# microsoft/OmniParser

Hardware: AMD Instinct MI355X
Metric: screenshots/sec end-to-end (detect+caption) @1920x1080 (higher is better)
Workload: dtype f32 (split-f16x3 MFMA)

## Files before the change

### omniparser_amd/csrc/gemm_dma.hip

```cpp
#include "omni_internal.h"
#include "gemm_common.h"
#include <string.h>
#include <type_traits>

OMNI_RANGE_GUARD_TU()

namespace {

typedef __attribute__((address_space(3))) void lds_void;

struct GemmArgs {
  const unsigned char* x; const unsigned char* w; const float* bias; const float* res; unsigned char* y;
  int M, N, K, nk;
  int ldi, in_coff, ldo, out_coff, ldr, res_coff;
  int mtiles, ntiles, xcd_order, xcd_n;
  float oscale;
  int img_tiles; unsigned w_img_stride; const float* img_oscale;
};

#if defined(__AMDGCN__)
struct RowBuf {
  __amdgpu_buffer_rsrc_t r;
  __device__ __forceinline__ RowBuf(const void* base, unsigned bytes) : r(__builtin_amdgcn_make_buffer_rsrc((void*)base, 0, (int)bytes, 0x00020000)) {}
  __device__ __forceinline__ void store16(unsigned off, f32x4 v) const { __builtin_amdgcn_raw_buffer_store_b128(__builtin_bit_cast(u32x4, v), r, (int)off, 0, 0); }
  __device__ __forceinline__ f32x4 load16(unsigned off) const { return __builtin_bit_cast(f32x4, __builtin_amdgcn_raw_buffer_load_b128(r, (int)off, 0, 0)); }
};
#else
struct RowBuf {
  unsigned char* base; unsigned bytes;
  RowBuf(const void* b, unsigned n) : base((unsigned char*)b), bytes(n) {}
  void store16(unsigned off, f32x4 v) const { if (off + 16u <= bytes) *reinterpret_cast<f32x4*>(base + off) = v; }
  f32x4 load16(unsigned off) const { return off + 16u <= bytes ? *reinterpret_cast<const f32x4*>(base + off) : f32x4{0.f, 0.f, 0.f, 0.f}; }
};
#endif

template <int BM, int BN, int WM, int WN, int TM, int TN, int LDS_BYTES, int ACT, bool OSPLIT, bool RES>
__device__ __forceinline__ void gemm_epilogue(f32x16 (&acc)[TM][TN], const GemmArgs& a, unsigned char* lds, int m0, int n0, int wave, int lane, float osc) {
  constexpr int NW = WM * WN;
  const int wm = wave / WN, wn = wave % WN;
  const int hsel = lane >> 5;
  static_assert(TN % 2 == 0, "epilogue stages 64 channels (256 bytes per row) of a wave at a time");
  constexpr int EP = 272;
  static_assert(NW * 32 * EP <= LDS_BYTES, "epilogue staging must fit the LDS ring");
  __syncthreads();
  unsigned char* stg = lds + wave * (32 * EP);
  float amax = 0.0f;
  const int rrow = lane >> 4, chunk = lane & 15;
  const int trows = min(a.M - m0, BM), wc0 = n0 + wn * (BN / WN);
  const RowBuf ybuf(a.y + ((long long)m0 * a.ldo + a.out_coff + wc0) * 4, (unsigned)(trows - 1) * (unsigned)(a.ldo * 4) + (BN / WN) * 4);
  const RowBuf rbuf(RES ? reinterpret_cast<const unsigned char*>(a.res) + ((long long)m0 * a.ldr + a.res_coff + wc0) * 4 : a.y,
// ... 36 lines not shown
            for (int c = 0; c < 4; c += 2) {
              f32x2 t = __builtin_elementwise_fma(f32x2{ac[q * 4 + c], ac[q * 4 + c + 1]}, (f32x2)osc, f32x2{bq[j][q][c], bq[j][q][c + 1]});
              if constexpr (ACT == OMNI_ACT_SILU) t = f32x2{t[0] / (1.0f + expf(-t[0])), t[1] / (1.0f + expf(-t[1]))};
              v[c] = t[0]; v[c + 1] = t[1];
            }
          }
          const int cl = j * 32 + q * 8 + 4 * hsel;
          if constexpr (OSPLIT) {
            uint2 hi, lo;
            omni_split4(v, hi, lo, amax);
            *reinterpret_cast<uint2*>(wr + omni_split_off(cl)) = hi;
            *reinterpret_cast<uint2*>(wr + omni_split_off(cl) + 32) = lo;
          } else {
            *reinterpret_cast<f32x4*>(wr + cl * 4) = f32x4{v[0], v[1], v[2], v[3]};
          }
        }
      OMNI_WAVE_SYNC();
      f32x4 ov[8];
#pragma unroll
      for (int it = 0; it < 8; ++it) {
        ov[it] = *reinterpret_cast<const f32x4*>(stg + (it * 4 + rrow) * EP + chunk * 16);
        if constexpr (RES) ov[it] += rres[it];
      }
      if constexpr (RES) { if (i + 1 < TM) load_res(i + 1); }
#pragma unroll
      for (int it = 0; it < 8; ++it) ybuf.store16(yoff + (unsigned)(i * 32 + it * 4) * (unsigned)(a.ldo * 4) + jh * 256, ov[it]);
      OMNI_WAVE_SYNC();
      __builtin_amdgcn_sched_barrier(0);
    }
  }
  if constexpr (OSPLIT) omni_report_range(amax);
}

template <int BM, int BN, int WM, int WN, int NSTAGE, int ACT, bool OSPLIT, bool RES, int SCHED = 0>
__global__ __launch_bounds__(WM * WN * 64, 2) void gemm_dma_kernel(GemmArgs a) {
#if defined(__HIP_DEVICE_COMPILE__)
  constexpr int NW = WM * WN;
  constexpr int TM = BM / (32 * WM), TN = BN / (32 * WN);
  constexpr int A_DMA = BM / (8 * NW), B_DMA = BN / (8 * NW);
  constexpr int DPS = A_DMA + B_DMA;
  constexpr int STAGE = (BM + BN) * 128;
  constexpr int NP = TM / 2;
  constexpr int NU = 2 * NP;
  constexpr int NM = 6 * TN;
  static_assert(TM % 2 == 0 && TN >= 1 && A_DMA >= 1 && B_DMA >= 1 && NSTAGE >= 2 && NSTAGE <= 4, "tile / wave grid mismatch");
  static_assert(BM * 128 + (TN - 1) * 4096 < 65536 && (TM - 1) * 4096 < 65536, "ds_read immediate offsets");
  __shared__ __attribute__((aligned(16))) unsigned char lds[NSTAGE * STAGE];

  const int tid = threadIdx.x, lane = tid & 63;
  const int wave = __builtin_amdgcn_readfirstlane(tid >> 6);
  const int wm = wave / WN, wn = wave % WN;
  int mt, nt;
  if (!tile_of_block(blockIdx.x, a.mtiles, a.ntiles, a.xcd_order, a.xcd_n, mt, nt)) return;
  const int m0 = __builtin_amdgcn_readfirstlane(mt) * BM, n0 = __builtin_amdgcn_readfirstlane(nt) * BN;
  const int img = a.img_tiles ? __builtin_amdgcn_readfirstlane(mt / a.img_tiles) : 0;
  const float osc = a.img_oscale ? a.img_oscale[img] : a.oscale;

  const int rsub = lane >> 3, slot = lane & 7;
  unsigned voffA[A_DMA], voffB[B_DMA];
  auto pieceA = [&](int i) { return SCHED == 2 ? wave + NW * i : wave * A_DMA + i; };
#pragma unroll
  for (int i = 0; i < A_DMA; ++i) {
    const int rl = pieceA(i) * 8 + rsub;
    const int rr = min(rl, a.M - 1 - m0);
    voffA[i] = (unsigned)rr * (unsigned)(a.ldi * 4) + (unsigned)((slot ^ ((rl >> 1) & 7)) * 16);
  }
#pragma unroll
  for (int i = 0; i < B_DMA; ++i) {
    const int rl = (wave * B_DMA + i) * 8 + rsub;
    const int rr = min(rl, a.N - 1 - n0);
    voffB[i] = (unsigned)rr * (unsigned)(a.K * 4) + (unsigned)((slot ^ ((rl >> 1) & 7)) * 16);
  }
  const __amdgpu_buffer_rsrc_t rsrcA =
      __builtin_amdgcn_make_buffer_rsrc((void*)(a.x + ((long long)m0 * a.ldi + a.in_coff) * 4), 0, 0x7fffffff, 0x00020000);
  const __amdgpu_buffer_rsrc_t rsrcB =
      __builtin_amdgcn_make_buffer_rsrc((void*)(a.w + (long long)img * a.w_img_stride + (long long)n0 * a.K * 4), 0, 0x7fffffff, 0x00020000);
  auto issue_piece = [&](int kt, int stage, int i) {
    const int so = kt * 128;
    if (i < A_DMA)
      __builtin_amdgcn_raw_ptr_buffer_load_lds(rsrcA, (lds_void*)(lds + stage * STAGE + pieceA(i) * 1024), 16, voffA[i], so, 0, 0);
    else
      __builtin_amdgcn_raw_ptr_buffer_load_lds(rsrcB, (lds_void*)(lds + stage * STAGE + BM * 128 + (wave * B_DMA + i - A_DMA) * 1024), 16,
                                               voffB[i - A_DMA], so, 0, 0);
  };
  auto issue = [&](int kt, int stage) {
#pragma unroll
    for (int i = 0; i < DPS; ++i) issue_piece(kt, stage, i);
  };

  const int swz = (lane >> 1) & 7, hsel = lane >> 5;
  int offA[4], offW[4];
#pragma unroll
  for (int gp = 0; gp < 4; ++gp) {
    const int c = ((((gp >> 1) * 4 + (gp & 1) * 2 + hsel) ^ swz)) * 16;
    offA[gp] = (wm * (BM / WM) + (lane & 31)) * 128 + c;
    offW[gp] = BM * 128 + (wn * (BN / WN) + (lane & 31)) * 128 + c;
  }
  struct AF { f16x8 h[2], l[2]; };
  struct WF { f16x8 h[TN], l[TN]; };
  auto loadA = [&](const unsigned char* st, int g, int ip, AF& f) {
#pragma unroll
    for (int t = 0; t < 2; ++t) {
      f.h[t] = *reinterpret_cast<const f16x8*>(st + offA[g * 2 + 0] + (ip * 2 + t) * 4096);
      f.l[t] = *reinterpret_cast<const f16x8*>(st + offA[g * 2 + 1] + (ip * 2 + t) * 4096);
    }
  };
  auto loadW = [&](const unsigned char* st, int g, WF& f) {
#pragma unroll
    for (int j = 0; j < TN; ++j) {
      f.h[j] = *reinterpret_cast<const f16x8*>(st + offW[g * 2 + 0] + j * 4096);
      f.l[j] = *reinterpret_cast<const f16x8*>(st + offW[g * 2 + 1] + j * 4096);
    }
  };

  f32x16 acc[TM][TN];
#pragma unroll
  for (int i = 0; i < TM; ++i)
#pragma unroll
    for (int j = 0; j < TN; ++j)
#pragma unroll
// ... 30 lines not shown
    constexpr bool MORE = decltype(more_tag)::value;
    if constexpr (NSTAGE > 2 && MORE) OMNI_WAIT_VMCNT((NSTAGE - 2) * DPS);
    else OMNI_WAIT_VMCNT(0);
    __builtin_amdgcn_s_barrier();
    const unsigned char* st = lds + stage * STAGE;
    loadW(st, 0, wf[0]);
    loadA(st, 0, 0, af[0]);
#pragma unroll
    for (int u = 0; u < NU; ++u) {
      const int g = u / NP, ip = u % NP;
      int nds = 0;
      if (u + 1 < NU) {
        const int g2 = (u + 1) / NP, ip2 = (u + 1) % NP;
        if (g2 != g) { loadW(st, g2, wf[g2 & 1]); nds += 2 * TN; }
        loadA(st, g2, ip2, af[(u + 1) & 1]);
        nds += 4;
      }
      if constexpr (MORE) {
#pragma unroll
        for (int i = u * PPU; i < (u + 1) * PPU && i < DPS; ++i) issue_piece(kt + NSTAGE - 1, nstage, i);
      }
      mma(af[u & 1], wf[g & 1], ip);
      {
        const int npc = (MORE && u < IU) ? PPU : 0;
#pragma unroll
        for (int k = 0; k < NM; ++k) {
          __builtin_amdgcn_sched_group_barrier(0x8, 1, 0);
          if (k < nds) __builtin_amdgcn_sched_group_barrier(0x100, 1, 0);
          else if (k < nds + npc) __builtin_amdgcn_sched_group_barrier(0x20, 1, 0);
        }
      }
      __builtin_amdgcn_sched_barrier(0);
    }
    stage = stage + 1 == NSTAGE ? 0 : stage + 1;
    nstage = nstage + 1 == NSTAGE ? 0 : nstage + 1;
  };
  if constexpr (SCHED == 2) {
    static_assert(BM == 256 && BN == 256 && WM == 2 && WN == 4 && NSTAGE == 2 && TM == 4 && TN == 2 && A_DMA == 4 && B_DMA == 4, "ping-pong: 256x256 tile, 8 waves");
    OMNI_WAIT_VMCNT(0);
    __builtin_amdgcn_s_barrier();
    if (wm == 1) __builtin_amdgcn_s_barrier();
    auto phase_barrier = [&]() {
      __builtin_amdgcn_sched_barrier(0);
      __builtin_amdgcn_s_barrier();
      __builtin_amdgcn_sched_barrier(0);
    };
    {
      AF afp;
      auto slice_pp = [&](int kt, auto more_tag) {
        constexpr bool MORE = decltype(more_tag)::value;
        const unsigned char* st = lds + stage * STAGE;
#pragma unroll
        for (int u = 0; u < 4; ++u) {
          const int g = u & 1, ip = u >> 1;
          if (u < 2) loadW(st, g, wf[g]);
          loadA(st, g, ip, afp);
          if constexpr (MORE) {
            if (u == 0) { issue_piece(kt + 1, nstage, 0); issue_piece(kt + 1, nstage, 2); }
            if (u == 1) { issue_piece(kt + 1, nstage, A_DMA + 0); issue_piece(kt + 1, nstage, A_DMA + 1); }
            if (u == 2) { issue_piece(kt + 1, nstage, A_DMA + 2); issue_piece(kt + 1, nstage, A_DMA + 3); }
            if (u == 3) { issue_piece(kt + 1, nstage, 1); issue_piece(kt + 1, nstage, 3); }
            if (u == 1) OMNI_WAIT_VMCNT(4);
            if (u == 3) OMNI_WAIT_VMCNT(2);
          } else {
            if (u == 1) OMNI_WAIT_VMCNT(0);
          }
          phase_barrier();
          __builtin_amdgcn_s_setprio(1);
          mma(afp, wf[g], ip);
          __builtin_amdgcn_s_setprio(0);
          phase_barrier();
        }
        stage ^= 1;
        nstage ^= 1;
      };
      int ktp = 0;
      for (; ktp + 1 < nk; ++ktp) slice_pp(ktp, std::true_type{});
      for (; ktp < nk; ++ktp) slice_pp(ktp, std::false_type{});
    }
    if (wm == 0) __builtin_amdgcn_s_barrier();
  } else {
  int kt = 0;
  for (; kt + NSTAGE - 1 < nk; ++kt) slice(kt, std::true_type{});
  for (; kt < nk; ++kt) slice(kt, std::false_type{});
  }

  gemm_epilogue<BM, BN, WM, WN, TM, TN, NSTAGE * STAGE, ACT, OSPLIT, RES>(acc, a, lds, m0, n0, wave, lane, osc);
#endif
}

__global__ __launch_bounds__(256) void split_convert_kernel(const float* __restrict__ x, unsigned char* __restrict__ y, long long rows,
                                                            int C, int ldi, int in_coff, int ldo, int out_coff) {
  const int gpr = C / 16;
  const long long idx = (long long)blockIdx.x * blockDim.x + threadIdx.x;
  if (idx >= rows * gpr) return;
  const long long r = idx / gpr;
  const int g = (int)(idx - r * gpr);
  const float* src = x + r * ldi + in_coff + g * 16;
  f32x4 v[4];
#pragma unroll
  for (int q = 0; q < 4; ++q) v[q] = *reinterpret_cast<const f32x4*>(src + q * 4);
  uint2 hi[4], lo[4];
#pragma unroll
  for (int q = 0; q < 4; ++q) {
    float t[4] = {v[q][0], v[q][1], v[q][2], v[q][3]};
// ... 111 lines not shown
        float v[4];
#pragma unroll
        for (int r = 0; r < 4; r += 2) {
          const f32x2 t = omni_gelu2(__builtin_elementwise_fma(f32x2{a1[0][q * 4 + r], a1[0][q * 4 + r + 1]} + f32x2{a1[1][q * 4 + r], a1[1][q * 4 + r + 1]},
                                                               (f32x2)osc1, f32x2{bq[r], bq[r + 1]}));
          v[r] = t[0]; v[r + 1] = t[1];
        }
        omni_split4(v, hq[qq], lq[qq], amax);
      }
      gh[kg] = __builtin_bit_cast(f16x8, u32x4{hq[0].x, hq[0].y, hq[1].x, hq[1].y});
      gl[kg] = __builtin_bit_cast(f16x8, u32x4{lq[0].x, lq[0].y, lq[1].x, lq[1].y});
    }
#pragma unroll
    for (int kg = 0; kg < 2; ++kg)
#pragma unroll
      for (int j = 0; j < OB; j += 2) {
        const unsigned char* sw = st + W1B + j * 4096;
        const f16x8 wh0 = *reinterpret_cast<const f16x8*>(sw + fo[kg][0]), wl0 = *reinterpret_cast<const f16x8*>(sw + fo[kg][1]);
        const f16x8 wh1 = *reinterpret_cast<const f16x8*>(sw + 4096 + fo[kg][0]), wl1 = *reinterpret_cast<const f16x8*>(sw + 4096 + fo[kg][1]);
        acc2[0][j] = __builtin_amdgcn_mfma_f32_32x32x16_f16(wh0, gh[kg], acc2[0][j], 0, 0, 0);
        acc2[0][j + 1] = __builtin_amdgcn_mfma_f32_32x32x16_f16(wh1, gh[kg], acc2[0][j + 1], 0, 0, 0);
        acc2[0][j] = __builtin_amdgcn_mfma_f32_32x32x16_f16(wl0, gh[kg], acc2[0][j], 0, 0, 0);
        acc2[0][j + 1] = __builtin_amdgcn_mfma_f32_32x32x16_f16(wl1, gh[kg], acc2[0][j + 1], 0, 0, 0);
        acc2[0][j] = __builtin_amdgcn_mfma_f32_32x32x16_f16(wh0, gl[kg], acc2[0][j], 0, 0, 0);
        acc2[0][j + 1] = __builtin_amdgcn_mfma_f32_32x32x16_f16(wh1, gl[kg], acc2[0][j + 1], 0, 0, 0);
      }
  }
  omni_report_range(amax);
  gemm_epilogue<NW * 32, C, NW, 1, 1, OB, 2 * STAGE, OMNI_ACT_NONE, false, true>(acc2, a.ep, lds, m0, 0, wave, lane, a.ep.oscale);
#endif
}

template <int BM, int BN, int WM, int WN, int NSTAGE>
int launch_tile(GemmArgs& a, int rows_per_img, int act, int osplit, hipStream_t s) {
  if (rows_per_img % BM != 0) {
    omni_set_error("gemm_dma: per-image weights need whole %d-row tiles per image (rows per image %d)", BM, rows_per_img);
    return OMNI_E_ARG;
  }
  a.img_tiles = rows_per_img / BM;
  a.mtiles = (a.M + BM - 1) / BM;
  a.ntiles = a.N / BN;
  a.xcd_order = (a.mtiles >= 64 && a.ntiles > 1) ? 1 : 0;
  a.xcd_n = a.xcd_order ? choose_xcd_n(a.ntiles, 4ll * a.N * a.K) : 1;
  dim3 grid(tile_grid(a.mtiles, a.ntiles, a.xcd_order, a.xcd_n)), block(WM * WN * 64);
  const bool res = a.res != nullptr;
  constexpr int SCHED1 = (BM == 256 && BN == 256) ? 1 : 0;
  const char* sched_e = getenv("OMNI_GEMM_SCHED");
  const bool lockstep = sched_e && atoi(sched_e) == 1;
#define OMNI_GD(ACT_, OS_, RES_)                                                                                                   \
  do {                                                                                                                             \
    if constexpr (BM == 256 && BN == 256) {                                                                                        \
      if (!lockstep) { hipLaunchKernelGGL((gemm_dma_kernel<BM, BN, WM, WN, NSTAGE, ACT_, OS_, RES_, 2>), grid, block, 0, s, a); break; }  \
    }                                                                                                                              \
    hipLaunchKernelGGL((gemm_dma_kernel<BM, BN, WM, WN, NSTAGE, ACT_, OS_, RES_, SCHED1>), grid, block, 0, s, a);                  \
  } while (0)
  if (act == OMNI_ACT_NONE && !osplit && !res) OMNI_GD(OMNI_ACT_NONE, false, false);
  else if (act == OMNI_ACT_NONE && !osplit && res) OMNI_GD(OMNI_ACT_NONE, false, true);
  else if (act == OMNI_ACT_NONE && osplit && !res) OMNI_GD(OMNI_ACT_NONE, true, false);
  else if (act == OMNI_ACT_GELU && osplit && !res) OMNI_GD(OMNI_ACT_GELU, true, false);
  else if (act == OMNI_ACT_GELU && !osplit && !res) OMNI_GD(OMNI_ACT_GELU, false, false);
#undef OMNI_GD
  else {
    omni_set_error("gemm_dma: unsupported epilogue (act %d, split out %d, residual %d)", act, osplit, (int)res);
    return OMNI_E_ARG;
  }
  return OMNI_OK;
}

}

int omni_launch_gemm_dma(const omni_op_t* op, hipStream_t s) {
  GemmArgs a{};
  a.x = (const unsigned char*)op->p[0]; a.w = (const unsigned char*)op->p[1]; a.bias = (const float*)op->p[2];
  a.res = (const float*)op->p[3]; a.y = (unsigned char*)op->p[4];
  const int B = op->i[0], H = op->i[1], W = op->i[2];
  a.K = op->i[3]; a.ldi = op->i[4]; a.in_coff = op->i[5];
  a.N = op->i[12]; a.ldo = op->i[13]; a.out_coff = op->i[14];
  const int act = op->i[15];
  a.ldr = op->i[16]; a.res_coff = op->i[17];
  const int osplit = op->i[21];
  a.oscale = op->f[1] != 0.0f ? op->f[1] : 1.0f;
  OMNI_REQUIRE(op->dtype == OMNI_F32, "gemm_dma: f32 plans only");
  OMNI_REQUIRE(a.x && a.w && a.y, "gemm_dma: null pointer");
  OMNI_REQUIRE(op->i[6] == 1 && op->i[7] == 1 && op->i[8] == 1 && op->i[9] == 0 && op->i[10] == H && op->i[11] == W,
               "gemm_dma: pointwise layers only");
  OMNI_REQUIRE(op->f[0] == 0.0f, "gemm_dma: output scale is not supported");
  const long long M = (long long)B * H * W;
  OMNI_REQUIRE(M > 0 && M < (1ll << 31), "gemm_dma: bad M");
  a.M = (int)M;
  OMNI_REQUIRE(a.K >= 32 && a.K % 32 == 0 && a.N % 128 == 0, "gemm_dma: needs K %% 32 == 0 and N %% 128 == 0 (K %d, N %d)", a.K, a.N);
  OMNI_REQUIRE(a.ldi % 16 == 0 && a.in_coff % 16 == 0, "gemm_dma: split input needs 16-channel aligned ld / offset (%d, %d)", a.ldi, a.in_coff);
  OMNI_REQUIRE(a.ldo % 4 == 0 && a.out_coff % 4 == 0 && (!osplit || (a.ldo % 16 == 0 && a.out_coff % 16 == 0)), "gemm_dma: output alignment");
  OMNI_REQUIRE(!a.res || (a.ldr % 4 == 0 && a.res_coff % 4 == 0), "gemm_dma: residual alignment");
  OMNI_REQUIRE((long long)a.ldi * 4 * 256 < (1ll << 31) && (long long)a.K * 4 * 256 < (1ll << 31) && (long long)a.ldo * 4 * 256 < (1ll << 31) &&
               (long long)a.ldr * 4 * 256 < (1ll << 31), "gemm_dma: row stride too large");
  a.nk = a.K / 32;
  const int rows_per_img = op->i[26];
  OMNI_REQUIRE(rows_per_img >= 0 && op->i[27] >= 0, "gemm_dma: bad per-image weight arguments (%d rows, stride %d)", rows_per_img, op->i[27]);
  if (rows_per_img > 0) {
    OMNI_REQUIRE(a.M % rows_per_img == 0, "gemm_dma: %d rows are no whole number of images of %d rows", a.M, rows_per_img);
    OMNI_REQUIRE(op->i[27] % 16 == 0 && (op->i[27] == 0 || op->i[27] >= a.N * a.K * 4), "gemm_dma: per-image weight stride %d (N %d, K %d)", op->i[27], a.N, a.K);
    a.w_img_stride = (unsigned)op->i[27];
    a.img_oscale = (const float*)op->p[6];
  }
  int tile = (a.N % 256 == 0) ? 0 : 1;
  {
    const long long mt256 = (a.M + 255) / 256;
    if (mt256 * (a.N / (tile == 0 ? 256 : 128)) < 256) tile = (tile == 0 && mt256 * (a.N / 128) >= 256) ? 1 : 2;
  }
  if (const char* e = getenv("OMNI_GEMM_TILE")) {
    if (!strcmp(e, "256x128")) tile = 1;
    else if (!strcmp(e, "128x128")) tile = 2;
    else if (!strcmp(e, "256x256") && a.N % 256 == 0) tile = 0;
  }
  int rc;
  if (tile == 0) rc = launch_tile<256, 256, 2, 4, 2>(a, rows_per_img, act, osplit, s);
  else if (tile == 1) rc = launch_tile<256, 128, 4, 2, 3>(a, rows_per_img, act, osplit, s);
  else rc = launch_tile<128, 128, 2, 2, 2>(a, rows_per_img, act, osplit, s);
  if (rc) return rc;
  OMNI_HIP_CHECK(hipGetLastError());
  return OMNI_OK;
}

int omni_launch_split_convert(const omni_op_t* op, hipStream_t s) {
  const long long rows = (long long)op->i[0] * (op->i[1] > 0 ? op->i[1] : 1);
  const int C = op->i[3], ldi = op->i[4], in_coff = op->i[5], ldo = op->i[13], out_coff = op->i[14];
  OMNI_REQUIRE(op->dtype == OMNI_F32 && op->p[0] && op->p[4], "split_convert: f32 plans, non-null pointers");
  OMNI_REQUIRE(rows > 0 && C > 0 && C % 16 == 0 && ldi % 16 == 0 && in_coff % 16 == 0 && ldo % 16 == 0 && out_coff % 16 == 0,
               "split_convert: 16-channel alignment (C %d, ld %d/%d, off %d/%d)", C, ldi, ldo, in_coff, out_coff);
  const long long total = rows * (C / 16);
  hipLaunchKernelGGL(split_convert_kernel, dim3((unsigned)((total + 255) / 256)), dim3(256), 0, s, (const float*)op->p[0],
                     (unsigned char*)op->p[4], rows, C, ldi, in_coff, ldo, out_coff);
  OMNI_HIP_CHECK(hipGetLastError());
  return OMNI_OK;
}

int omni_launch_mlp_fused(const omni_op_t* op, hipStream_t s) {
  MlpArgs a{};
  a.x = (const unsigned char*)op->p[0]; a.w1 = (const unsigned char*)op->p[1]; a.b1 = (const float*)op->p[2];
  a.w2 = (const unsigned char*)op->p[5];
  a.ep.x = nullptr; a.ep.w = nullptr; a.ep.bias = (const float*)op->p[6]; a.ep.res = (const float*)op->p[3]; a.ep.y = (unsigned char*)op->p[4];
  const long long M = (long long)op->i[0] * (op->i[1] > 0 ? op->i[1] : 1);
  const int C = op->i[3], HID = op->i[12];
  a.ldi = op->i[4]; a.in_coff = op->i[5];
  a.ep.ldo = op->i[13]; a.ep.out_coff = op->i[14]; a.ep.ldr = op->i[16]; a.ep.res_coff = op->i[17];
  a.osc1 = op->f[1] != 0.0f ? op->f[1] : 1.0f;
  a.ep.oscale = op->f[2] != 0.0f ? op->f[2] : 1.0f;
  OMNI_REQUIRE(op->dtype == OMNI_F32, "mlp_fused: f32 plans only");
  OMNI_REQUIRE(a.x && a.w1 && a.w2 && a.b1 && a.ep.bias && a.ep.res && a.ep.y, "mlp_fused: null pointer (both biases and the residual are required)");
  OMNI_REQUIRE(C == 128 && HID == 512, "mlp_fused: built for C = 128, hidden = 512 (got %d, %d)", C, HID);
  OMNI_REQUIRE(M > 0 && M < (1ll << 31), "mlp_fused: bad row count");
// ... 11 lines not shown
```

### omniparser_amd/florence.py

```python
import json
import math
import os
from pathlib import Path
from types import SimpleNamespace
from typing import Dict, List, Optional

import numpy as np
import torch

from . import _lib as L
from .planner import PlanBuilder, View, torch_dtype

PROMPT_IDS = [0, 2264, 473, 5, 2274, 6190, 116, 2]
TEXT_CAPACITIES = (8, 16, 32, 64)


def text_capacity(n_tokens: int) -> int:
    for c in TEXT_CAPACITIES:
        if n_tokens <= c:
            return c
    raise ValueError(f"a prompt of {n_tokens} tokens exceeds the captioner's limit of {TEXT_CAPACITIES[-1]} prompt tokens "
                     "(bos and eos included)")


# ... 537 lines not shown
                                  y2=y2.ptr if y2 is not None else None, period=period, omode=omode, eps=eps))
            out.fmt = "split" if omode == 1 else "f32"
            if y2 is not None:
                y2.fmt = "split"
            return out

        def dwconv(key, x: View, out: View):
            wp, bp = W.dwconv(key)
            pb.keep += [wp, bp]
            pb.add_op(L.make_op(L.OP_DWCONV3, dt, p=[x.ptr, wp.data_ptr(), bp.data_ptr(), None, out.ptr],
                                i={0: x.B, 1: x.H, 2: x.W, 3: x.C}))
            return out

        fuse_env = cap.fuse_dwln
        attn_split = use_dma and cap.attn_split_out

        def dwconv_ln(conv_key, norm_key, x: View, y1: View, hout: View):
            if not (fuse_env and dt == L.F32 and x.C in (128, 256, 512)):
                dwconv(conv_key, x, y1)
                return layernorm(norm_key, y1, hout, split=hout)
            wp, bp = W.dwconv(conv_key)
            pb.keep += [wp, bp]
            pb.add_op(L.make_op(L.OP_DWCONV3_LN, dt,
                                p=[x.ptr, wp.data_ptr(), bp.data_ptr(), hout.ptr, y1.ptr,
                                   W.f32(norm_key + ".weight").data_ptr(), W.f32(norm_key + ".bias").data_ptr()],
                                i={0: x.B, 1: x.H, 2: x.W, 3: x.C, 6: 1 if grp["dma"] else 0}, f={0: 1e-5}))
            hout.fmt = "split" if grp["dma"] else "f32"
            return hout

        self.x_in = pb.alloc(B, R, R, V, zero=True)
        x = self.x_in
        vt = "model.vision_tower."
        self.chan_ws = None
        self.fold_stages = []
        self.stage_out = []
        for s in range(4):
            C = w.embed_dim[s]
            grp["dma"] = use_dma and C % 128 == 0
            k, st, pd = w.patch[s]
            Ho = (x.H + 2 * pd - k) // st + 1
            conv_key = f"{vt}convs.{s}.conv"
            if w.prenorm[s]:
                xn = pb.alloc(B, x.H, x.W, x.C)
                layernorm(f"{vt}convs.{s}.norm", x, xn)
                cur = pb.alloc(B, Ho, Ho, C)
                wp, bp = W.packed(conv_key, lambda: (sd[conv_key + ".weight"], sd[conv_key + ".bias"]))
                pb.conv(xn, wp, bp, cur, k, st, pd)
                pb.release(xn, *([] if x is self.x_in else [x]))
            else:
                t0 = pb.alloc(B, Ho, Ho, C)
                if cap.patch_rows and dt == L.F32 and pb.split and V == 4 and k <= 8 and x is self.x_in:
                    wp, bp = W.cached((conv_key, dt, "patch"), lambda: (pb.pack_weight_patch(sd[conv_key + ".weight"], V),
                                                                         pb.upload(sd[conv_key + ".bias"].float())))
                    pb.conv_patch(x, wp, bp, t0, k, st, pd)
                else:
                    wp, bp = W.cached((conv_key, dt, "pad"), lambda: (pb.pack_weight(sd[conv_key + ".weight"], cin_pad=V),
                                                                       pb.upload(sd[conv_key + ".bias"].float())))
                    pb.conv(x, wp, bp, t0, k, st, pd)
                cur = pb.alloc(B, Ho, Ho, C)
                layernorm(f"{vt}convs.{s}.norm", t0, cur)
                pb.release(t0)
            H = Ho
            N = H * H
            A_, B_ = cur, pb.alloc(B, H, H, C)
            hbuf = pb.alloc(B, H, H, C)
            qkv = pb.alloc(B, H, H, 3 * C)
            att = pb.alloc(B, H, H, C)
            mlp_one = grp["dma"] and cap.fuse_mlp and C == 128 and sd[f"{vt}blocks.{s}.0.spatial_block.ffn.fc1.weight"].shape[0] == 512
            ffn = None if mlp_one else pb.alloc(B, H, H, 4 * C)
            chunk_tokens = 1024
            chunks = (N + chunk_tokens - 1) // chunk_tokens
            cws = pb.raw((B * w.groups[s] * chunks * 1024,), torch.float32, zero=False)
            fold = bool(cap.fold_chan_proj) and grp["dma"] and dt == L.F32 and C % 128 == 0 and N % 256 == 0 and N >= 4 * C
            fold_wf = fold_wb = fold_sc = fold_mx = None
            if fold:
                fold_wf = pb.raw((B * C * C,), torch.float32, zero=False)
                fold_wb = pb.raw((B * C * C,), torch.float32, zero=False)
                fold_sc = pb.raw((B,), torch.float32, zero=False)
                fold_mx = pb.raw((B * (C // 64) * w.groups[s],), torch.float32, zero=False)
# ... 147 lines not shown
        self.prompt_ids[:n].copy_(ids.expand(n, -1), non_blocking=True)
        self.nkeys[:n].copy_(nkeys.expand(n), non_blocking=True)

    def rows_for(self, cap: "Florence2Captioner", n: int) -> int:
        last, cap._last_remainder = getattr(cap, "_last_remainder", None), n
        if n in self._row_plans or n == last:
            return n
        return min(cap.bucket(n), self.B)

    def encode_rows(self, cap: "Florence2Captioner", n: int, stream=None) -> "_CaptionPlans":
        assert self.arena is None and 1 <= n <= self.B
        if n == self.B:
            return self
        cp = self._row_plans.pop(n, None)
        if cp is None:
            while len(self._row_plans) >= max(1, int(cap.row_graphs)):
                if dev_sync := (cap.device.type == "cuda"):
                    torch.cuda.synchronize(cap.device)
                self._row_plans.pop(next(iter(self._row_plans)))
            cp = _CaptionPlans(cap, n, self.R, self.T - 1, arena=self, stream=stream)
            cap.row_graph_builds = getattr(cap, "row_graph_builds", 0) + 1
        self._row_plans[n] = cp
        return cp


class _Config(SimpleNamespace):
    pass


class Florence2Captioner:
    fuse_dwln = True
    attn_split_out = True
    fold_chan_proj = True
    fuse_mlp = True
    exact_rows = os.environ.get("OMNI_EXACT_ROWS", "1") != "0"
    row_graphs = int(os.environ.get("OMNI_CAPTION_ROW_GRAPHS", "24"))
    patch_rows = os.environ.get("OMNI_PATCH_ROWS", "1") != "0"
    reuse_activations = True

    long_kv_budget_bytes = 2 ** 30

    def __init__(self, model_dir, device=None, precision: Optional[str] = None, resolution: Optional[int] = None):
        device = L.require_device(device, "Florence2Captioner")
        L.lib()
        self.device = device
        precision = precision or os.environ.get("OMNI_PRECISION", "f32")
        self.dtype = L.F32 if precision == "f32" else L.F16
        self.resolution = int(resolution or os.environ.get("OMNI_CAPTION_RES", "768"))
        self.w = FlorenceWeights(model_dir)
        self.config = _Config(name_or_path=str(model_dir) if "florence" in str(model_dir).lower() else f"florence:{model_dir}",
                              model_type="florence2")
        self.use_graph = os.environ.get("OMNI_HIPGRAPH", "1") != "0"
        self.stream = self._lane_stream(0)
        self._wcache = {}
        self._plans = {}
        self.max_new_tokens = 20
        self.early_exit_every = 5
        self.num_beams = 1
        self.token_scores = False
        self.last_steps = 0
        self._lut, self._bic = None, {}
        self._lock = L.DeviceLock(self.device, reentrant=True)

    def to(self, *a, **k):
        return self

# ... 461 lines not shown
```

### omniparser_amd/opwork.py

```python

NAMES = {1: "conv_igemm/conv_split", 2: "avgpool2", 3: "maxpool", 4: "resize_nearest", 5: "letterbox", 6: "detect_decode", 7: "nms",
         8: "dwconv3", 9: "layernorm", 10: "attn_rows (window / MHA)", 11: "chan_attn", 12: "proj_prep", 13: "assemble", 14: "embed_step",
         15: "attn_decode", 16: "greedy_step", 17: "crop_resize", 18: "dwconv3_ln", 19: "split_convert", 20: "hand_off", 21: "overlay",
         22: "png_pack", 23: "png_deflate", 24: "mlp_fused"}

MFMA_KINDS = (1, 24, 10)


def op_work(op, esz=4):
    i = op.i
    k = op.kind
    if k == 1:
        M, N, K = i[0] * i[10] * i[11], i[12], i[6] * i[7] * i[3]
        if i[25]:
            K = i[6] * i[6] * i[4]
            return 2 * M * N * K, esz * (i[0] * i[1] * i[2] * i[4] + N * K + M * N)
        nw = M // i[26] if (i[20] == 2 and i[26] > 0) else 1
        return 2 * M * N * K, esz * (i[0] * i[1] * i[2] * i[3] + nw * N * K + M * N * (2 if op.p[3] else 1))
    if k == 24:
        rows, C, hid = i[0] * max(i[1], 1), i[3], i[12]
        return 4 * rows * C * hid, esz * (3 * rows * C + 2 * C * hid)
    if k in (2, 3, 4):
        return 0, esz * (i[0] * i[1] * i[2] * i[3] + i[0] * max(i[10], 1) * max(i[11], 1) * i[3])
    if k in (8, 18):
# ... 11 lines not shown
            return 2 * B * N * C * 32 + 2 * B * C * C * 32, esz * (B * N * C * 2 + C * C + B * C * C)
        return 4 * B * N * C * 32, esz * B * N * C * 4
    if k == 15:
        B, heads, nk = i[10], i[6], (i[7] if i[7] > 0 else i[8])
        return 4 * B * heads * nk * 64, esz * B * nk * i[9] * 2
    if k == 16:
        return 0, esz * i[0] * i[1]
    return 0, 0


def op_shape(op):
    i, k = op.i, op.kind
    if k in (1, 19):
        return (i[0] * max(i[10], 1) * max(i[11], 1) if k == 1 else i[0] * max(i[1], 1), i[12] if k == 1 else i[3], i[6] * i[7] * i[3] if k == 1 else 0)
    if k == 24:
        return (i[0] * max(i[1], 1), i[3], i[12])
    if k in (8, 18):
        return (i[0] * i[1] * i[2], i[3], 0)
    if k == 9:
        return (i[0] * max(i[1], 1), i[3], i[6])
    if k == 10:
        return (i[11] * i[9], i[8] * i[15], i[12])
    if k == 11:
        return (i[0] * i[1], i[3], 1 if i[8] == 1 else 0)
    if k == 15:
        return (i[10], i[9], i[7] if i[7] > 0 else i[8])
    return (i[0], i[3], 0)


def op_kernel(op):
    if op.kind == 1:
        if op.i[20] == 2 and op.i[26] > 0:
            return "gemm_dma (per-image weights)"
        return "gemm_dma" if op.i[20] == 2 else ("conv_split" if op.i[20] else "conv_igemm")
    if op.kind == 11 and op.i[8] == 1:
        return "chan_attn (scores + fold)"
    return NAMES.get(op.kind, str(op.kind))
```

### omniparser_amd/planner.py

```python
import math
import os
from dataclasses import dataclass
from typing import Optional

import torch

from . import _lib as L


def vec_width(dtype: int) -> int:
    return 4 if dtype == L.F32 else 8


def torch_dtype(dtype: int):
    return torch.float32 if dtype == L.F32 else torch.float16


@dataclass
class View:
    t: torch.Tensor
    coff: int
    C: int
    fmt: str = "f32"

# ... 142 lines not shown
        self.reused_bytes += need
        return block[:need].view(dtype).view(shape)

    def upload(self, host_tensor: torch.Tensor) -> torch.Tensor:
        t = host_tensor.contiguous().to(self.device)
        self.keep.append(_register(t, "const"))
        return t

    @staticmethod
    def split_f16(w2d: torch.Tensor) -> torch.Tensor:
        cout, K = w2d.shape
        assert K % 16 == 0
        w2d = w2d.float().clamp(-65504.0, 65504.0)
        hi = w2d.to(torch.float16)
        lo = ((w2d - hi.float()) * 2048.0).to(torch.float16)
        return torch.cat([hi.view(cout, K // 16, 16), lo.view(cout, K // 16, 16)], -1).contiguous()

    @staticmethod
    def split_f16_b(w2d: torch.Tensor):
        cout, K = w2d.shape
        assert K % 16 == 0
        w2d = w2d.double()
        amax = float(w2d.abs().max())
        k = 0 if amax == 0.0 else 12 - math.floor(math.log2(amax))
        k = max(-24, min(24, k))
        ws = (w2d * (2.0 ** k)).float()
        hi = ws.to(torch.float16)
        lo = (ws - hi.float()).to(torch.float16)
        return torch.cat([hi.view(cout, K // 16, 16), lo.view(cout, K // 16, 16)], -1).contiguous(), 2.0 ** -k

    KPERM16 = (0, 1, 2, 3, 8, 9, 10, 11, 4, 5, 6, 7, 12, 13, 14, 15)

    def pack_weight_dma(self, w: torch.Tensor, kperm: bool = False) -> torch.Tensor:
        w2d = w.detach().float().reshape(w.shape[0], -1)
        if kperm:
            cout, K = w2d.shape
            assert K % 16 == 0
            w2d = w2d.view(cout, K // 16, 16)[:, :, list(self.KPERM16)].reshape(cout, K).contiguous()
        t, oscale = self.split_f16_b(w2d)
        t = self.upload(t)
        t.omni_fmt, t.omni_oscale = 2, oscale
        return t

    def pack_weight(self, w: torch.Tensor, cin_pad: Optional[int] = None) -> torch.Tensor:
        w = w.detach().float()
        cout, cin, kh, kw = w.shape
        if cin_pad and cin_pad > cin:
            w = torch.cat([w, w.new_zeros(cout, cin_pad - cin, kh, kw)], 1)
        w = w.permute(0, 2, 3, 1).reshape(cout, -1)
        cin_eff = max(cin, cin_pad or 0)
        if self.split and self.dtype == L.F32 and cin_eff % 32 == 0 and cin_eff * kh * kw >= 128:
            t = self.upload(self.split_f16(w))
            t.omni_fmt = 1
            return t
        return self.upload(w.to(torch_dtype(self.dtype)))

    def conv(self, x: View, w_packed: torch.Tensor, bias: Optional[torch.Tensor], out: View, k: int, s: int = 1,
             p: Optional[int] = None, act: int = L.ACT_NONE, res: Optional[View] = None, scale: float = 0.0,
             out_split: bool = False):
        p = k // 2 if p is None else p
        Ho = (x.H + 2 * p - k) // s + 1
        Wo = (x.W + 2 * p - k) // s + 1
        assert (out.B, out.H, out.W) == (x.B, Ho, Wo), ((out.B, out.H, out.W), (x.B, Ho, Wo))
        cout = out.C
        wfmt = getattr(w_packed, "omni_fmt", 0) if self.dtype == L.F32 else 0
        if wfmt:
            assert w_packed.dtype == torch.float16 and w_packed.numel() == 2 * cout * k * k * x.C and x.C % 32 == 0, \
                (tuple(w_packed.shape), cout, k, x.C)
        else:
            assert tuple(w_packed.shape) == (cout, k * k * x.C), (tuple(w_packed.shape), cout, k, x.C)
        if wfmt == 2:
            assert k == 1 and s == 1 and p == 0 and scale == 0.0 and cout % 128 == 0, "format-B weights: pointwise layers, Cout % 128 == 0"
            assert x.fmt == "split", "the LDS-DMA GEMM reads a pre-split input: its producer must emit format B (or insert split_convert)"
            assert x.ld % 16 == 0 and x.coff % 16 == 0 and not (out_split and (res is not None or out.ld % 16 or out.coff % 16))
        else:
            assert x.fmt == "f32" and not out_split, "register-staged conv kernels read and write f32"
        if res is not None:
            assert (res.B, res.H, res.W, res.C) == (out.B, out.H, out.W, out.C) and res.fmt == "f32"
        b = None
        if bias is not None:
            b = bias if bias.device == self.device and bias.dtype == torch.float32 else self.upload(bias.detach().float())
            ent = _TENSORS.get(b.data_ptr())
            if ent is None or ent[0]() is not b:
                _register(b, "const")
            self.keep.append(b)
            assert b.numel() == cout
        if self.ws is None and (self.device.type == "cuda" or self.workspace_on_host):
            self.ws = self.raw((self.ws_kib * 256,), torch.float32, zero=False)
        if self.cnt is None and self.ws is not None and self.n_cnt and wfmt == 1:
            self.cnt = self.raw((self.n_cnt,), torch.int32, zero=True)
        cnt = self.cnt if (wfmt == 1 and self.cnt is not None) else None
        tune = (0, 0)
        if wfmt == 1 and self.conv_tuning:
            tune = tuple(self.conv_tuning.get(conv_key(x.B * Ho * Wo, cout, k * k * x.C, k, s), (0, 0)))
        op = L.make_op(
            L.OP_CONV, self.dtype,
            p=[x.ptr, w_packed.data_ptr(), b.data_ptr() if b is not None else None,
               res.ptr if res is not None else None, out.ptr, self.ws.data_ptr() if self.ws is not None else None,
               cnt.data_ptr() if cnt is not None else None],
            i={0: x.B, 1: x.H, 2: x.W, 3: x.C, 4: x.ld, 5: x.coff, 6: k, 7: k, 8: s, 9: p, 10: Ho, 11: Wo,
               12: cout, 13: out.ld, 14: out.coff, 15: act,
               16: res.ld if res is not None else 0, 17: res.coff if res is not None else 0,
               19: self.ws_kib if self.ws is not None else 0, 20: wfmt, 21: 1 if out_split else 0,
               22: tune[0], 23: tune[1], 24: cnt.numel() if cnt is not None else 0},
            f={0: scale, 1: getattr(w_packed, "omni_oscale", 0.0) if wfmt == 2 else 0.0})
# ... 143 lines not shown
```

Before: 12.83.

## Run 3x3 stride-2 downsampling convs through the LDS-DMA implicit GEMM

Extends the LDS-DMA split-f16 GEMM kernel with an implicit-GEMM mode for 3x3 stride-2 pad-1 convolutions. The A-tile offsets walk the input window per K-chunk, and padding rows and columns are zero-filled through an out-of-range buffer offset. The Florence vision tower's downsampling convs now use this path by default, with a split_convert inserted after the layernorm. The aim is to replace the slower register-staged conv kernel with the pipelined DMA GEMM, at the cost of an extra split-conversion pass and more complex address logic.

```diff
diff --git a/omniparser_amd/csrc/gemm_dma.hip b/omniparser_amd/csrc/gemm_dma.hip
--- a/omniparser_amd/csrc/gemm_dma.hip
+++ b/omniparser_amd/csrc/gemm_dma.hip
@@ -16,6 +16,7 @@
   int mtiles, ntiles, xcd_order, xcd_n;
   float oscale;
   int img_tiles; unsigned w_img_stride; const float* img_oscale;
+  int cW, cHo, cWo, cCS;
 };
 
 #if defined(__AMDGCN__)
@@ -118,7 +119,7 @@
   if constexpr (OSPLIT) omni_report_range(amax);
 }
 
-template <int BM, int BN, int WM, int WN, int NSTAGE, int ACT, bool OSPLIT, bool RES, int SCHED = 0>
+template <int BM, int BN, int WM, int WN, int NSTAGE, int ACT, bool OSPLIT, bool RES, int SCHED = 0, bool CONV = false>
 __global__ __launch_bounds__(WM * WN * 64, 2) void gemm_dma_kernel(GemmArgs a) {
 #if defined(__HIP_DEVICE_COMPILE__)
   constexpr int NW = WM * WN;
@@ -145,11 +146,23 @@
   const int rsub = lane >> 3, slot = lane & 7;
   unsigned voffA[A_DMA], voffB[B_DMA];
   auto pieceA = [&](int i) { return SCHED == 2 ? wave + NW * i : wave * A_DMA + i; };
+  unsigned cpad = 0;
+  int cp0 = 0;
+  if constexpr (CONV) {
+    const int r0 = m0 / a.cWo;
+    cp0 = __builtin_amdgcn_readfirstlane(2 * a.cW * r0 + 2 * (m0 - r0 * a.cWo));
+  }
 #pragma unroll
   for (int i = 0; i < A_DMA; ++i) {
     const int rl = pieceA(i) * 8 + rsub;
     const int rr = min(rl, a.M - 1 - m0);
-    voffA[i] = (unsigned)rr * (unsigned)(a.ldi * 4) + (unsigned)((slot ^ ((rl >> 1) & 7)) * 16);
+    if constexpr (CONV) {
+      const int m = m0 + rr, r = m / a.cWo, xo = m - r * a.cWo, yo = r % a.cHo;
+      voffA[i] = (unsigned)(2 * a.cW * r + 2 * xo - cp0) * (unsigned)(a.ldi * 4) + (unsigned)((slot ^ ((rl >> 1) & 7)) * 16);
+      cpad |= ((yo == 0 ? 1u : 0u) | (xo == 0 ? 2u : 0u)) << (2 * i);
+    } else {
+      voffA[i] = (unsigned)rr * (unsigned)(a.ldi * 4) + (unsigned)((slot ^ ((rl >> 1) & 7)) * 16);
+    }
   }
 #pragma unroll
   for (int i = 0; i < B_DMA; ++i) {
@@ -157,21 +170,45 @@
     const int rr = min(rl, a.N - 1 - n0);
     voffB[i] = (unsigned)rr * (unsigned)(a.K * 4) + (unsigned)((slot ^ ((rl >> 1) & 7)) * 16);
   }
-  const __amdgpu_buffer_rsrc_t rsrcA =
-      __builtin_amdgcn_make_buffer_rsrc((void*)(a.x + ((long long)m0 * a.ldi + a.in_coff) * 4), 0, 0x7fffffff, 0x00020000);
+  const __amdgpu_buffer_rsrc_t rsrcA = __builtin_amdgcn_make_buffer_rsrc(
+      (void*)(a.x + ((long long)(CONV ? cp0 - a.cW - 1 : m0) * a.ldi + a.in_coff) * 4), 0, 0x7fffffff, 0x00020000);
   const __amdgpu_buffer_rsrc_t rsrcB =
       __builtin_amdgcn_make_buffer_rsrc((void*)(a.w + (long long)img * a.w_img_stride + (long long)n0 * a.K * 4), 0, 0x7fffffff, 0x00020000);
+  int c_so = 0, c_cs = 0, c_dx = 0;
+  unsigned c_pm = 3;
+  auto conv_next = [&]() {
+    const bool wcs = c_cs + 1 == a.cCS, wdx = wcs && c_dx == 2;
+    c_so += wcs ? (a.ldi - a.cCS * 32) * 4 + 128 : 128;
+    c_so += wdx ? (a.cW - 3) * a.ldi * 4 : 0;
+    c_cs = wcs ? 0 : c_cs + 1;
+    c_pm = wdx ? 2u : (wcs ? 0u : c_pm & 2u) | (c_pm & 1u);
+    c_dx = wcs ? (wdx ? 0 : c_dx + 1) : c_dx;
+  };
   auto issue_piece = [&](int kt, int stage, int i) {
     const int so = kt * 128;
-    if (i < A_DMA)
-      __builtin_amdgcn_raw_ptr_buffer_load_lds(rsrcA, (lds_void*)(lds + stage * STAGE + pieceA(i) * 1024), 16, voffA[i], so, 0, 0);
-    else
+    if (i < A_DMA) {
+      if constexpr (CONV) {
+#if defined(__AMDGCN__)
+        __builtin_amdgcn_raw_ptr_buffer_load_lds(rsrcA, (lds_void*)(lds + stage * STAGE + pieceA(i) * 1024), 16,
+                                                 (cpad & (c_pm << (2 * i))) ? 0x80000000u : voffA[i], c_so, 0, 0);
+#else
+        static const unsigned char zeros[16] = {};
+        if (cpad & (c_pm << (2 * i)))
+          __builtin_amdgcn_raw_ptr_buffer_load_lds(__builtin_amdgcn_make_buffer_rsrc((void*)zeros, 0, 16, 0x00020000),
+                                                   (lds_void*)(lds + stage * STAGE + pieceA(i) * 1024), 16, 0u, 0, 0, 0);
+        else
+          __builtin_amdgcn_raw_ptr_buffer_load_lds(rsrcA, (lds_void*)(lds + stage * STAGE + pieceA(i) * 1024), 16, voffA[i], c_so, 0, 0);
+#endif
+      } else
+        __builtin_amdgcn_raw_ptr_buffer_load_lds(rsrcA, (lds_void*)(lds + stage * STAGE + pieceA(i) * 1024), 16, voffA[i], so, 0, 0);
+    } else
       __builtin_amdgcn_raw_ptr_buffer_load_lds(rsrcB, (lds_void*)(lds + stage * STAGE + BM * 128 + (wave * B_DMA + i - A_DMA) * 1024), 16,
                                                voffB[i - A_DMA], so, 0, 0);
   };
   auto issue = [&](int kt, int stage) {
 #pragma unroll
     for (int i = 0; i < DPS; ++i) issue_piece(kt, stage, i);
+    if constexpr (CONV) conv_next();
   };
 
   const int swz = (lane >> 1) & 7, hsel = lane >> 5;
@@ -268,6 +305,7 @@
       }
       __builtin_amdgcn_sched_barrier(0);
     }
+    if constexpr (CONV && MORE) conv_next();
     stage = stage + 1 == NSTAGE ? 0 : stage + 1;
     nstage = nstage + 1 == NSTAGE ? 0 : nstage + 1;
   };
@@ -307,6 +345,7 @@
           __builtin_amdgcn_s_setprio(0);
           phase_barrier();
         }
+        if constexpr (CONV && MORE) conv_next();
         stage ^= 1;
         nstage ^= 1;
       };
@@ -484,7 +523,7 @@
 }
 
 template <int BM, int BN, int WM, int WN, int NSTAGE>
-int launch_tile(GemmArgs& a, int rows_per_img, int act, int osplit, hipStream_t s) {
+int launch_tile(GemmArgs& a, int rows_per_img, int act, int osplit, bool conv, hipStream_t s) {
   if (rows_per_img % BM != 0) {
     omni_set_error("gemm_dma: per-image weights need whole %d-row tiles per image (rows per image %d)", BM, rows_per_img);
     return OMNI_E_ARG;
@@ -506,6 +545,19 @@
     }                                                                                                                              \
     hipLaunchKernelGGL((gemm_dma_kernel<BM, BN, WM, WN, NSTAGE, ACT_, OS_, RES_, SCHED1>), grid, block, 0, s, a);                  \
   } while (0)
+  if (conv) {
+    if (act != OMNI_ACT_NONE || osplit || res) {
+      omni_set_error("gemm_dma: the 3x3 stride-2 form has no activation, format-B output or residual (act %d, split out %d, residual %d)", act, osplit, (int)res);
+      return OMNI_E_ARG;
+    }
+    if constexpr (BM == 256 && BN == 256) {
+      if (!lockstep) hipLaunchKernelGGL((gemm_dma_kernel<BM, BN, WM, WN, NSTAGE, OMNI_ACT_NONE, false, false, 2, true>), grid, block, 0, s, a);
+      else hipLaunchKernelGGL((gemm_dma_kernel<BM, BN, WM, WN, NSTAGE, OMNI_ACT_NONE, false, false, SCHED1, true>), grid, block, 0, s, a);
+    } else {
+      hipLaunchKernelGGL((gemm_dma_kernel<BM, BN, WM, WN, NSTAGE, OMNI_ACT_NONE, false, false, SCHED1, true>), grid, block, 0, s, a);
+    }
+    return OMNI_OK;
+  }
   if (act == OMNI_ACT_NONE && !osplit && !res) OMNI_GD(OMNI_ACT_NONE, false, false);
   else if (act == OMNI_ACT_NONE && !osplit && res) OMNI_GD(OMNI_ACT_NONE, false, true);
   else if (act == OMNI_ACT_NONE && osplit && !res) OMNI_GD(OMNI_ACT_NONE, true, false);
@@ -526,7 +578,8 @@
   a.x = (const unsigned char*)op->p[0]; a.w = (const unsigned char*)op->p[1]; a.bias = (const float*)op->p[2];
   a.res = (const float*)op->p[3]; a.y = (unsigned char*)op->p[4];
   const int B = op->i[0], H = op->i[1], W = op->i[2];
-  a.K = op->i[3]; a.ldi = op->i[4]; a.in_coff = op->i[5];
+  const int Cin = op->i[3];
+  a.K = Cin; a.ldi = op->i[4]; a.in_coff = op->i[5];
   a.N = op->i[12]; a.ldo = op->i[13]; a.out_coff = op->i[14];
   const int act = op->i[15];
   a.ldr = op->i[16]; a.res_coff = op->i[17];
@@ -534,10 +587,25 @@
   a.oscale = op->f[1] != 0.0f ? op->f[1] : 1.0f;
   OMNI_REQUIRE(op->dtype == OMNI_F32, "gemm_dma: f32 plans only");
   OMNI_REQUIRE(a.x && a.w && a.y, "gemm_dma: null pointer");
-  OMNI_REQUIRE(op->i[6] == 1 && op->i[7] == 1 && op->i[8] == 1 && op->i[9] == 0 && op->i[10] == H && op->i[11] == W,
-               "gemm_dma: pointwise layers only");
+  const bool conv = !(op->i[6] == 1 && op->i[7] == 1);
+  int Ho = H, Wo = W;
+  if (conv) {
+    OMNI_REQUIRE(op->i[6] == 3 && op->i[7] == 3 && op->i[8] == 2 && op->i[9] == 1,
+                 "gemm_dma: pointwise layers, or 3x3 / stride 2 / pad 1 (k %dx%d, stride %d, pad %d)", op->i[6], op->i[7], op->i[8], op->i[9]);
+    OMNI_REQUIRE(B > 0 && H >= 2 && W >= 2 && H % 2 == 0 && W % 2 == 0 && op->i[10] == H / 2 && op->i[11] == W / 2,
+                 "gemm_dma: the 3x3 stride-2 form needs even H and W and Ho = H / 2, Wo = W / 2 (H %d, W %d, Ho %d, Wo %d)", H, W, op->i[10], op->i[11]);
+    OMNI_REQUIRE(Cin >= 32 && Cin % 32 == 0 && Cin <= a.ldi - a.in_coff, "gemm_dma: the 3x3 stride-2 form needs Cin %% 32 == 0 (Cin %d, ld %d, offset %d)", Cin, a.ldi, a.in_coff);
+    OMNI_REQUIRE(op->i[26] == 0 && op->i[27] == 0, "gemm_dma: per-image weights are pointwise only");
+    OMNI_REQUIRE((long long)B * H * W < (1ll << 31), "gemm_dma: image tensor too large");
+    Ho = H / 2; Wo = W / 2;
+    a.K = 9 * Cin;
+    a.cW = W; a.cHo = Ho; a.cWo = Wo; a.cCS = Cin / 32;
+    OMNI_REQUIRE(((long long)2 * W * (255 / Wo + 2) + 4ll * W + 8) * a.ldi * 4 < (1ll << 31), "gemm_dma: a tile's input window exceeds 2 GB (W %d, ld %d)", W, a.ldi);
+  } else {
+    OMNI_REQUIRE(op->i[8] == 1 && op->i[9] == 0 && op->i[10] == H && op->i[11] == W, "gemm_dma: pointwise layers, or 3x3 / stride 2 / pad 1");
+  }
   OMNI_REQUIRE(op->f[0] == 0.0f, "gemm_dma: output scale is not supported");
-  const long long M = (long long)B * H * W;
+  const long long M = (long long)B * Ho * Wo;
   OMNI_REQUIRE(M > 0 && M < (1ll << 31), "gemm_dma: bad M");
   a.M = (int)M;
   OMNI_REQUIRE(a.K >= 32 && a.K % 32 == 0 && a.N % 128 == 0, "gemm_dma: needs K %% 32 == 0 and N %% 128 == 0 (K %d, N %d)", a.K, a.N);
@@ -566,9 +634,9 @@
     else if (!strcmp(e, "256x256") && a.N % 256 == 0) tile = 0;
   }
   int rc;
-  if (tile == 0) rc = launch_tile<256, 256, 2, 4, 2>(a, rows_per_img, act, osplit, s);
-  else if (tile == 1) rc = launch_tile<256, 128, 4, 2, 3>(a, rows_per_img, act, osplit, s);
-  else rc = launch_tile<128, 128, 2, 2, 2>(a, rows_per_img, act, osplit, s);
+  if (tile == 0) rc = launch_tile<256, 256, 2, 4, 2>(a, rows_per_img, act, osplit, conv, s);
+  else if (tile == 1) rc = launch_tile<256, 128, 4, 2, 3>(a, rows_per_img, act, osplit, conv, s);
+  else rc = launch_tile<128, 128, 2, 2, 2>(a, rows_per_img, act, osplit, conv, s);
   if (rc) return rc;
   OMNI_HIP_CHECK(hipGetLastError());
   return OMNI_OK;
diff --git a/omniparser_amd/florence.py b/omniparser_amd/florence.py
--- a/omniparser_amd/florence.py
+++ b/omniparser_amd/florence.py
@@ -593,6 +593,7 @@
         x = self.x_in
         vt = "model.vision_tower."
         self.chan_ws = None
+        self.conv_dma_stages = []
         self.fold_stages = []
         self.stage_out = []
         for s in range(4):
@@ -603,9 +604,14 @@
             conv_key = f"{vt}convs.{s}.conv"
             if w.prenorm[s]:
                 xn = pb.alloc(B, x.H, x.W, x.C)
+                conv_dma = (bool(cap.conv_dma) and use_dma and (k, st, pd) == (3, 2, 1) and x.C % 32 == 0 and C % 128 == 0
+                            and x.H % 2 == 0 and x.W % 2 == 0 and Ho * Ho >= 256)
+                self.conv_dma_stages += [s] if conv_dma else []
                 layernorm(f"{vt}convs.{s}.norm", x, xn)
+                if conv_dma:
+                    pb.split_convert(xn)
                 cur = pb.alloc(B, Ho, Ho, C)
-                wp, bp = W.packed(conv_key, lambda: (sd[conv_key + ".weight"], sd[conv_key + ".bias"]))
+                wp, bp = W.packed(conv_key, lambda: (sd[conv_key + ".weight"], sd[conv_key + ".bias"]), dma=conv_dma)
                 pb.conv(xn, wp, bp, cur, k, st, pd)
                 pb.release(xn, *([] if x is self.x_in else [x]))
             else:
@@ -819,6 +825,7 @@
     fuse_dwln = True
     attn_split_out = True
     fold_chan_proj = True
+    conv_dma = True
     fuse_mlp = True
     exact_rows = os.environ.get("OMNI_EXACT_ROWS", "1") != "0"
     row_graphs = int(os.environ.get("OMNI_CAPTION_ROW_GRAPHS", "24"))
diff --git a/omniparser_amd/opwork.py b/omniparser_amd/opwork.py
--- a/omniparser_amd/opwork.py
+++ b/omniparser_amd/opwork.py
@@ -67,6 +67,8 @@
     if op.kind == 1:
         if op.i[20] == 2 and op.i[26] > 0:
             return "gemm_dma (per-image weights)"
+        if op.i[20] == 2 and op.i[6] == 3:
+            return "gemm_dma (conv 3x3 s2)"
         return "gemm_dma" if op.i[20] == 2 else ("conv_split" if op.i[20] else "conv_igemm")
     if op.kind == 11 and op.i[8] == 1:
         return "chan_attn (scores + fold)"
diff --git a/omniparser_amd/planner.py b/omniparser_amd/planner.py
--- a/omniparser_amd/planner.py
+++ b/omniparser_amd/planner.py
@@ -198,6 +198,9 @@
     KPERM16 = (0, 1, 2, 3, 8, 9, 10, 11, 4, 5, 6, 7, 12, 13, 14, 15)
 
     def pack_weight_dma(self, w: torch.Tensor, kperm: bool = False) -> torch.Tensor:
+        if w.dim() == 4 and tuple(w.shape[2:]) != (1, 1):
+            assert tuple(w.shape[2:]) == (3, 3) and w.shape[1] % 32 == 0 and not kperm, tuple(w.shape)
+            w = w.detach().float().permute(0, 2, 3, 1)
         w2d = w.detach().float().reshape(w.shape[0], -1)
         if kperm:
             cout, K = w2d.shape
@@ -236,7 +239,10 @@
         else:
             assert tuple(w_packed.shape) == (cout, k * k * x.C), (tuple(w_packed.shape), cout, k, x.C)
         if wfmt == 2:
-            assert k == 1 and s == 1 and p == 0 and scale == 0.0 and cout % 128 == 0, "format-B weights: pointwise layers, Cout % 128 == 0"
+            assert scale == 0.0 and cout % 128 == 0, "format-B weights: Cout % 128 == 0, no output scale"
+            if (k, s, p) != (1, 1, 0):
+                assert (k, s, p) == (3, 2, 1) and x.H % 2 == 0 and x.W % 2 == 0 and act == L.ACT_NONE and res is None and not out_split, \
+                    "format-B weights: pointwise layers, or 3x3 / stride 2 / pad 1 over even H, W without activation / residual"
             assert x.fmt == "split", "the LDS-DMA GEMM reads a pre-split input: its producer must emit format B (or insert split_convert)"
             assert x.ld % 16 == 0 and x.coff % 16 == 0 and not (out_split and (res is not None or out.ld % 16 or out.coff % 16))
         else:
```

Result: no change. 12.90, median of 6 (+0.6%).
